# phuang1024/Starst3r

Hardware: AMD Instinct MI355X
Metric: 3DGS train iters/sec @ 1M Gaussians, 8x1080p views (higher is better)
Workload: dtype f32

## Files before the change

### starst3r_amd/csrc/api.hip

```cpp
#include <stdarg.h>

#include "common.h"

static thread_local char g_err[512] = "";

void st3r_set_error(const char* fmt, ...) {
    va_list ap;
    va_start(ap, fmt);
    vsnprintf(g_err, sizeof(g_err), fmt, ap);
    va_end(ap);
}

ST3R_EXPORT int st3r_version(void) { return ST3R_VERSION; }
ST3R_EXPORT const char* st3r_last_error(void) { return g_err; }

ST3R_EXPORT int st3r_ctx_create(int device, st3r_ctx** out) {
    ARG_CHECK(out);
    int ndev = 0;
    HIP_TRY(hipGetDeviceCount(&ndev));
    ARG_CHECK(device >= 0 && device < ndev);
    HIP_TRY(hipSetDevice(device));
    st3r_ctx* c = new (std::nothrow) st3r_ctx();
    if (!c) { st3r_set_error("out of host memory"); return ST3R_ERR_NOMEM; }
    memset(c, 0, sizeof(*c));
// ... 43 lines not shown
    *grown = 0;
    if (bytes == 0) bytes = 16;
    if (ctx->slot_bytes[slot] < bytes) {
        size_t want = bytes + bytes / 4;
        want = (want + 255) & ~(size_t)255;
        if (ctx->slot_ptr[slot]) {
            HIP_TRY(hipDeviceSynchronize());
            HIP_TRY(hipFree(ctx->slot_ptr[slot]));
            ctx->slot_ptr[slot] = nullptr; ctx->slot_bytes[slot] = 0;
        }
        hipError_t e = hipMalloc(&ctx->slot_ptr[slot], want);
        if (e != hipSuccess) {
            st3r_set_error("arena slot %d: hipMalloc(%zu) failed: %s", slot, want, hipGetErrorString(e));
            return ST3R_ERR_NOMEM;
        }
        ctx->slot_bytes[slot] = want;
        *grown = 1;
    }
    *out = ctx->slot_ptr[slot];
    return ST3R_OK;
}

ST3R_EXPORT int st3r_ctx_peek(st3r_ctx* ctx, void* stream, int which, void* dst, int64_t bytes) {
    ARG_CHECK(ctx && dst && bytes >= 0 && which >= 0 && which <= 10);
    static const int slots[11] = {SLOT_VALS_B, SLOT_OFFSETS, SLOT_SPLATS, SLOT_CUM,
                                  SLOT_MCMC_CUM, SLOT_MCMC_DEAD, SLOT_MCMC_SAMPLED, SLOT_MCMC_COUNT,
                                  SLOT_RGB, SLOT_ALPHA, SLOT_COUNTS};
    ARG_CHECK((size_t)bytes <= ctx->slot_bytes[slots[which]]);
    HIP_TRY(hipMemcpyAsync(dst, ctx->slot_ptr[slots[which]], (size_t)bytes, hipMemcpyDeviceToDevice,
                           (hipStream_t)stream));
    return ST3R_OK;
}

static const char* k_stage_names[STG_COUNT] = {"project", "scan", "emit", "sort", "offsets", "blend_fwd", "loss",
                                               "blend_bwd", "project_bwd", "adam", "sort_depth"};

ST3R_EXPORT const char* st3r_stage_name(int stage) {
    return (stage >= 0 && stage < STG_COUNT) ? k_stage_names[stage] : "";
}

static void prof_harvest_slot(st3r_ctx* ctx, int slot) {
    for (int st = 0; st < STG_COUNT; ++st) {
        if (!ctx->prof_used[slot][st]) continue;
        float ms = 0.f;
        if (hipEventSynchronize(ctx->prof_ev[slot][st][1]) == hipSuccess &&
            hipEventElapsedTime(&ms, ctx->prof_ev[slot][st][0], ctx->prof_ev[slot][st][1]) == hipSuccess) {
            ctx->prof_ms[st] += ms; ctx->prof_n[st] += 1;
        }
        ctx->prof_used[slot][st] = 0;
    }
// ... 43 lines not shown
        ctx->prof_ms[st] = 0; ctx->prof_n[st] = 0;
    }
    return ST3R_OK;
}

int st3r_isect_scan_impl(st3r_ctx* ctx, hipStream_t s, int64_t n_pairs, const int32_t* tiles, int32_t* cum,
                         int64_t* n_isects_host, const void* pack_rects, int rect32, uint64_t* pack_out,
                         int32_t** total_dev_out, int32_t* total_copy, int32_t* total_host);
int st3r_isect_emit_impl(hipStream_t s, int N, int C, const float* splats, const int32_t* cum, int tile_size,
                         int tile_w, int tile_h, int64_t* isect_ids, int32_t* flatten_ids);
int st3r_sort_impl(st3r_ctx* ctx, hipStream_t s, int64_t n, int end_bit, int64_t* keys_in, int32_t* vals_in,
                   int64_t* keys_out, int32_t* vals_out);
int st3r_isect_offsets_impl(hipStream_t s, int64_t n_isects, const int64_t* ids, int C, int tile_w, int tile_h,
                            int32_t* offsets);
int st3r_project_impl(st3r_ctx* ctx, hipStream_t s, int N, int C, const float* means, const float* quats, const float* scales,
                      const float* opacities, const float* sh, int sh_stride, const float* viewmats, const float* Ks,
                      const float* campos, int width, int height, int tile_size, float eps2d, float near_plane,
                      float far_plane, float radius_clip, float* splats, int32_t* tiles_per_gauss, double* reg_sums,
                      uint64_t* depth_keys, int32_t* depth_vals, int tight, uint32_t key_base, void* rects, int rect32,
                      int reg_overwrite, double* zero_ptr, int zero_n, uint32_t* krange);
int st3r_sort_depth_seg_impl(st3r_ctx* ctx, hipStream_t s, int64_t N, int C, uint32_t* keys_in, int32_t* vals_in,
                             uint32_t* keys_out, int32_t* vals_out, const uint32_t* krange);
int st3r_isect_emit_chain_impl(st3r_ctx* ctx, hipStream_t s, int N, int C, const int32_t* perm, const void* rects,
                               int rect32, int tile_w, int tile_h, uint32_t* tile_keys, int32_t* vals, int64_t cap);
int st3r_records_prepare_impl(hipStream_t s, int N, int C, const float* splats, int tile_size, int tile_w, int tile_h,
                              int tight, int32_t* tiles, uint64_t* depth_keys, int32_t* depth_vals, uint32_t key_base,
                              void* rects, int rect32);
int st3r_isect_offsets32_impl(hipStream_t s, int64_t n_isects, const uint32_t* keys, int C, int tile_w, int tile_h,
                              int32_t* offsets, const int32_t* n_dev);
int st3r_sort_depth_impl(st3r_ctx* ctx, hipStream_t s, int64_t n, int end_bit, uint64_t* keys_in, int32_t* vals_in,
                         uint64_t* keys_out, int32_t* vals_out);
int st3r_sort_depth32_impl(st3r_ctx* ctx, hipStream_t s, int64_t n, int end_bit, uint32_t* keys_in, int32_t* vals_in,
                           uint32_t* keys_out, int32_t* vals_out);
int st3r_sort_tile_impl(st3r_ctx* ctx, hipStream_t s, int64_t n, int end_bit, uint32_t* keys_in, int32_t* vals_in,
                        uint32_t* keys_out, int32_t* vals_out, const int32_t* n_dev);
int st3r_blend_fwd_impl(st3r_ctx* ctx, hipStream_t s, int C, int W, int H, int tile_w, int tile_h,
                        const float* splats, const int32_t* offsets, const int32_t* flat, int64_t n_isects,
                        float* rgb, float* alpha, int32_t* last_ids, bool for_backward, bool end_in_offsets);
int st3r_blend_bwd_impl(st3r_ctx* ctx, hipStream_t s, int C, int W, int H, int tile_w, int tile_h,
                        const float* splats, const int32_t* offsets, const int32_t* flat, int64_t n_isects,
                        const float* alpha, const int32_t* last_ids, const float* v_rgb, const float* v_alpha,
                        const int32_t* cum, const uint64_t* rects, const uint64_t* rectbase, int tight, int64_t n_pairs,
                        float* v_splats,
                        bool end_in_offsets, st3r_vtile_ref* defer);
int st3r_project_sh_bwd_impl(hipStream_t s, int N, int C, const float* means, const float* quats, const float* scales,
                             const float* opacities, const float* sh, int sh_stride, const float* viewmats,
                             const float* Ks, const float* campos, int width, int height, float eps2d,
// ... 144 lines not shown
        if (n_isects > 2147483647LL) n_isects = 2147483647LL;
        ctx->count_pending = 1; ctx->count_cap = n_isects;
        o->n_visible = -1; o->n_isects_ref = -1;
    } else {
        HIP_TRY(hipMemcpyAsync(ctx->pinned, total_dev, sizeof(int32_t), hipMemcpyDeviceToHost, s));
        if (reg_sums) HIP_TRY(hipMemcpyAsync(ctx->pinned + 1, reg_sums + 2, 2 * sizeof(double), hipMemcpyDeviceToHost, s));
        HIP_TRY(hipStreamSynchronize(s));
        n_isects = (int64_t)((int32_t*)ctx->pinned)[0];
        if (n_isects < 0) {
            st3r_set_error("more than 2^31 tile intersections in one call: split the views over more calls / GPUs");
            return ST3R_SPLIT_VIEWS;
        }
        o->n_visible = reg_sums ? (int64_t)((double*)ctx->pinned)[1] : -1;
        o->n_isects_ref = reg_sums ? (int64_t)((double*)ctx->pinned)[2] : n_isects;
        if (allow_async) { ctx->isect_hint = n_isects; ctx->hint_sig = sig; }
    }
    GET(SLOT_KEYS_A, uint32_t, n_isects, tkeys_a);
    GET(SLOT_KEYS_B, uint32_t, n_isects, tkeys_b);
    GET(SLOT_VALS_A, int32_t, n_isects, vals_a);
    GET(SLOT_VALS_B, int32_t, n_isects, vals_b);
    n_dev = total_dev;
    o->n_records = async ? -1 : n_isects;
    if (n_isects > 0) {
        st3r_prof_begin(ctx, s, STG_EMIT);
        rc = st3r_isect_emit_chain_impl(ctx, s, N, C, perm, rects, rect32, tile_w, tile_h, tkeys_a, vals_a, n_isects);
        st3r_prof_end(ctx, s, STG_EMIT);
        if (rc) return rc;
        const int end_bit = bit_length_u32((uint32_t)((int64_t)C * tile_w * tile_h - 1));
        st3r_prof_begin(ctx, s, STG_SORT);
        rc = st3r_sort_tile_impl(ctx, s, n_isects, end_bit, tkeys_a, vals_a, tkeys_b, vals_b, n_dev);
        st3r_prof_end(ctx, s, STG_SORT);
        if (rc) return rc;
    }
    st3r_prof_begin(ctx, s, STG_OFFSETS);
    rc = st3r_isect_offsets32_impl(s, n_isects, tkeys_b, C, tile_w, tile_h, offsets, n_dev);
    st3r_prof_end(ctx, s, STG_OFFSETS);
    if (rc) return rc;
    o->splats = splats; o->offsets = offsets; o->flat = vals_b; o->cum = cum; o->rects = rect32 ? nullptr : rects;
    o->rectbase = rectbase;
    o->n_isects = n_isects;
    o->tile_w = tile_w; o->tile_h = tile_h;
    return ST3R_OK;
}

__global__ void k_finalize_loss(int C, const double* __restrict__ sums, const double* __restrict__ reg_sums,
                                double inv_px, double inv_cnt, double w_l1, double w_ssim, double reg_views,
                                double opac_k, double scale_k, float* __restrict__ loss_out) {
    if (threadIdx.x == 0 && blockIdx.x == 0) {
        double loss = 0;
        for (int c = 0; c < C; ++c) loss += w_l1 * sums[2 * c] * inv_px + w_ssim * (1.0 - sums[2 * c + 1] * inv_cnt);
        loss += reg_views * (opac_k * reg_sums[0] + scale_k * reg_sums[1]);
        loss_out[0] = (float)loss;
    }
// ... 192 lines not shown
```

### starst3r_amd/csrc/common.h

```cpp
#pragma once
#include <hip/hip_runtime.h>
#include <stdint.h>
#include <stdio.h>
#include <string.h>

#include "../../include/st3r.h"

#define ST3R_EXPORT extern "C" __attribute__((visibility("default")))

void st3r_set_error(const char* fmt, ...);

#define HIP_TRY(expr)                                                                              \
    do {                                                                                           \
        hipError_t _e = (expr);                                                                    \
        if (_e != hipSuccess) {                                                                    \
            st3r_set_error("%s:%d: %s -> %s", __FILE__, __LINE__, #expr, hipGetErrorString(_e));   \
            return ST3R_ERR_HIP;                                                                   \
        }                                                                                          \
    } while (0)

#define ARG_CHECK(cond)                                                                    \
    do {                                                                                   \
        if (!(cond)) {                                                                     \
            st3r_set_error("%s:%d: invalid argument: %s", __FILE__, __LINE__, #cond);      \
// ... 28 lines not shown
    SLOT_DKEYS_B,
    SLOT_DVALS_A,
    SLOT_DVALS_B,
    SLOT_CUM_D,
    SLOT_NN_PART,
    SLOT_MCMC_CUM,
    SLOT_MCMC_DEAD,
    SLOT_MCMC_RANK,
    SLOT_MCMC_COUNT,
    SLOT_MCMC_SAMPLED,
    SLOT_MCMC_BINOMS,
    SLOT_REG_PART,
    SLOT_RECTS,
    SLOT_RECTS_D,
    SLOT_RECTBASE,
    SLOT_COUNTS,
    SLOT_PSTAGE,
    SLOT_GSTAGE,
    SLOT_ALIGN_CTL,
    SLOT_PAIR_TOUCH,
    SLOT_KRANGE_PART,
    SLOT_SCAN_CHAIN,
    SLOT_POSE_PART,
    SLOT_COUNT
};

enum Stage {
    STG_PROJECT = 0,
    STG_SCAN,
    STG_EMIT,
    STG_SORT,
    STG_OFFSETS,
    STG_BLEND_FWD,
    STG_LOSS,
    STG_BLEND_BWD,
    STG_PROJECT_BWD,
    STG_ADAM,
    STG_SORT_DEPTH,
    STG_COUNT
};
#define PROF_RING 64
#define ST3R_MAX_RANGES 8

#define ST3R_SPLIT_VIEWS 1000

struct st3r_vtile_ref { const int32_t* cum; const float* vtile; int stamp; unsigned vt_cap; const uint32_t* touch; };
// ... 44 lines not shown
```

### starst3r_amd/csrc/gs_isect.hip

```cpp
#include "common.h"
#include "tile_rect.h"

#define SCAN_THREADS 256
#define SCAN_ITEMS 16
#define SCAN_TILE (SCAN_THREADS * SCAN_ITEMS)

__device__ __forceinline__ int wave_incl_scan(int v) {
    const int lane = threadIdx.x & 63;
#pragma unroll
    for (int off = 1; off < 64; off <<= 1) {
        int t = __shfl_up(v, off);
        if (lane >= off) v += t;
    }
    return v;
}

__device__ __forceinline__ int block_incl_scan(int v, int* total) {
    __shared__ int wsum[4];
    const int lane = threadIdx.x & 63, w = threadIdx.x >> 6;
    int inc = wave_incl_scan(v);
    if (lane == 63) wsum[w] = inc;
    __syncthreads();
    int base = 0;
#pragma unroll
// ... 357 lines not shown
                              void* rects, int rect32) {
    const int64_t n_pairs = (int64_t)N * C;
    if (n_pairs == 0) return ST3R_OK;
    hipLaunchKernelGGL(k_records_prepare, dim3(ceil_div(n_pairs, 256)), dim3(256), 0, s, N, n_pairs,
                       (const float4*)splats, tile_size, tile_w, tile_h, tight, tiles, depth_keys, depth_vals, key_base,
                       rects, rect32);
    LAUNCH_CHECK();
    return ST3R_OK;
}


#ifndef EP
#define EP 1024
#endif
#define EPT (EP / 256)
#define ECH 4096

__device__ __forceinline__ void emit_item(int C, int bpc, int* c, int* k) {
    const int b = blockIdx.x;
    if ((C & 7) == 0) { const int j = b >> 3; *c = (b & 7) + 8 * (j / bpc); *k = j % bpc; }
    else { *c = b / bpc; *k = b % bpc; }
}

__global__ __launch_bounds__(256) void k_isect_gather(int N, int C, int bpc, const int32_t* __restrict__ perm,
                                                      const void* __restrict__ rects, int rect32,
                                                      void* __restrict__ rects_d, int32_t* __restrict__ wg_tiles) {
    int c, k;
    emit_item(C, bpc, &c, &k);
    const int t = threadIdx.x;
    const int64_t first = (int64_t)c * N + (int64_t)k * EP;
    const int np = (int)min((int64_t)EP, (int64_t)(c + 1) * N - first);
    int32_t pid[EPT];
#pragma unroll
    for (int j = 0; j < EPT; ++j) pid[j] = j * 256 + t < np ? perm[first + j * 256 + t] : -1;
    int sum = 0;
#pragma unroll
    for (int j = 0; j < EPT; ++j) {
        if (pid[j] >= 0) {
            const int64_t dst = first + j * 256 + t;
            if (rect32) {
                const uint32_t r = reinterpret_cast<const uint32_t*>(rects)[pid[j]];
                reinterpret_cast<uint32_t*>(rects_d)[dst] = r;
                sum += (int)((r >> 16) & 0xFFu) * (int)(r >> 24);
            } else {
                const uint64_t r = reinterpret_cast<const uint64_t*>(rects)[pid[j]];
                reinterpret_cast<uint64_t*>(rects_d)[dst] = r;
                sum += (int)((r >> 32) & 0xFFFF) * (int)(r >> 48);
            }
        }
    }
    int total;
    block_incl_scan(sum, &total);
    if (t == 0) wg_tiles[c * bpc + k] = total;
}

#define EMIT_SELF_BASE_MAX 16384
__global__ __launch_bounds__(1024) void k_isect_wg_scan(int n, const int32_t* __restrict__ wg_tiles,
                                                        long long* __restrict__ wg_base) {
    __shared__ long long s_wave[16];
    const int t = threadIdx.x, lane = t & 63, w = t >> 6;
    const int per = (n + 1023) / 1024;
    const int e0 = min(t * per, n), e1 = min(e0 + per, n);
    long long sum = 0;
    for (int e = e0; e < e1; ++e) sum += wg_tiles[e];
    long long inc = sum;
#pragma unroll
    for (int off = 1; off < 64; off <<= 1) {
        const long long o = __shfl_up(inc, off);
        if (lane >= off) inc += o;
    }
    if (lane == 63) s_wave[w] = inc;
    __syncthreads();
    long long base = 0;
#pragma unroll
    for (int i = 0; i < 16; ++i) base += i < w ? s_wave[i] : 0;
    long long run = base + inc - sum;
    for (int e = e0; e < e1; ++e) { wg_base[e] = run; run += wg_tiles[e]; }
}

__global__ __launch_bounds__(256) void k_isect_emit_d(int N, int C, int bpc, const int32_t* __restrict__ perm,
                                                      const void* __restrict__ rects_d, int rect32,
                                                      const long long* __restrict__ wg_base,
                                                      const int32_t* __restrict__ wg_tiles, int tile_w, int tile_h,
                                                      uint32_t* __restrict__ tile_keys, int32_t* __restrict__ vals,
                                                      int64_t cap) {
    __shared__ int s_end[EP];
    __shared__ uint32_t s_org[EP];
    __shared__ uint16_t s_w[EP];
    __shared__ int32_t s_pid[EP];
    __shared__ uint16_t s_own[ECH];
    __shared__ unsigned s_wmax[4];
    __shared__ long long s_bsum[4];
    int c, k;
    emit_item(C, bpc, &c, &k);
    const int t = threadIdx.x, lane = t & 63, w = t >> 6;
    long long bsum = 0;
    if (!wg_base) {
        const int nb4 = (c * bpc + k) >> 2;
        for (int i = t; i < nb4; i += 256) {
            const int4 v = reinterpret_cast<const int4*>(wg_tiles)[i];
            bsum += ((long long)v.x + v.y) + ((long long)v.z + v.w);
        }
        if (t < ((c * bpc + k) & 3)) bsum += wg_tiles[4 * nb4 + t];
    }
    const int64_t first = (int64_t)c * N + (int64_t)k * EP;
    const int np = (int)min((int64_t)EP, (int64_t)(c + 1) * N - first);
    int cnt[EPT];
#pragma unroll
    for (int j = 0; j < EPT; ++j) {
        const int e = j * 256 + t;
        int32_t pid = 0;
        uint32_t org = 0, rw = 0, rh = 0;
        if (e < np) {
            pid = perm[first + e];
            rect_load(rects_d, rect32, first + e, &org, &rw, &rh);
        }
        s_pid[e] = pid; s_org[e] = org; s_w[e] = (uint16_t)rw;
        cnt[j] = (int)(rw * rh);
    }
    int carry = 0;
#pragma unroll
    for (int j = 0; j < EPT; ++j) {
        int tot;
        const int inc = block_incl_scan(cnt[j], &tot);
        s_end[j * 256 + t] = carry + inc;
        carry += tot;
    }
    const int total = carry;
    __syncthreads();
    long long base;
    if (wg_base) base = wg_base[c * bpc + k];
    else {
#pragma unroll
        for (int off = 32; off > 0; off >>= 1) bsum += __shfl_down(bsum, off);
        if (lane == 0) s_bsum[w] = bsum;
        __syncthreads();
        base = (s_bsum[0] + s_bsum[1]) + (s_bsum[2] + s_bsum[3]);
    }
    const uint32_t key0 = (uint32_t)c * (uint32_t)(tile_w * tile_h);
    int carry_owner = 0;
    for (int c0 = 0; c0 < total; c0 += ECH) {
        reinterpret_cast<uint4*>(s_own)[t] = make_uint4(0u, 0u, 0u, 0u);
        reinterpret_cast<uint4*>(s_own)[t + 256] = make_uint4(0u, 0u, 0u, 0u);
        __syncthreads();
#pragma unroll
        for (int j = 0; j < EPT; ++j) {
            const int e = j * 256 + t;
            if (e < np) {
                const int start = e ? s_end[e - 1] : 0;
                if (s_end[e] > start && start >= c0 && start < c0 + ECH) s_own[start - c0] = (uint16_t)(e + 1);
            }
        }
        __syncthreads();
        uint4 a = reinterpret_cast<const uint4*>(s_own)[2 * t], b = reinterpret_cast<const uint4*>(s_own)[2 * t + 1];
        unsigned wv[8] = {a.x, a.y, a.z, a.w, b.x, b.y, b.z, b.w};
        unsigned run = 0;
#pragma unroll
        for (int i = 0; i < 8; ++i) {
            const unsigned lo = max(run, wv[i] & 0xFFFFu);
            run = max(lo, wv[i] >> 16);
            wv[i] = lo | (run << 16);
        }
        unsigned inc = run;
#pragma unroll
        for (int off = 1; off < 64; off <<= 1) {
            const unsigned o = __shfl_up(inc, off);
            if (lane >= off) inc = max(inc, o);
        }
        if (lane == 63) s_wmax[w] = inc;
        unsigned excl_m = __shfl_up(inc, 1);
        if (lane == 0) excl_m = 0;
        __syncthreads();
        unsigned pre = max((unsigned)carry_owner, excl_m);
#pragma unroll
        for (int ww = 0; ww < 4; ++ww)
            if (ww < w) pre = max(pre, s_wmax[ww]);
        carry_owner = (int)max(max(max((unsigned)carry_owner, s_wmax[0]), max(s_wmax[1], s_wmax[2])), s_wmax[3]);
#pragma unroll
        for (int i = 0; i < 8; ++i) {
            const unsigned lo = max(wv[i] & 0xFFFFu, pre), hi = max(wv[i] >> 16, pre);
            wv[i] = lo | (hi << 16);
        }
        reinterpret_cast<uint4*>(s_own)[2 * t] = make_uint4(wv[0], wv[1], wv[2], wv[3]);
        reinterpret_cast<uint4*>(s_own)[2 * t + 1] = make_uint4(wv[4], wv[5], wv[6], wv[7]);
        __syncthreads();
        const int lim = min(ECH, total - c0);
        for (int i = t; i < lim; i += 256) {
            const int p = (int)s_own[i] - 1;
            const int o = c0 + i;
            const int kk = o - (p == 0 ? 0 : s_end[p - 1]);
            const uint32_t w_ = s_w[p], org = s_org[p];
            int qq = (int)((float)kk * __builtin_amdgcn_rcpf((float)w_));
            int rem = kk - qq * (int)w_;
            if (rem < 0) { --qq; rem += (int)w_; }
            if (rem >= (int)w_) { ++qq; rem -= (int)w_; }
            const uint32_t tx = (org & 0xFFFF) + (uint32_t)rem, ty = (org >> 16) + (uint32_t)qq;
            const long long pos = base + o;
            if (pos >= 0 && pos < cap) {
                tile_keys[pos] = key0 + ty * (uint32_t)tile_w + tx;
                vals[pos] = s_pid[p];
            }
        }
        __syncthreads();
    }
}

int st3r_isect_emit_chain_impl(st3r_ctx* ctx, hipStream_t s, int N, int C, const int32_t* perm, const void* rects,
                               int rect32, int tile_w, int tile_h, uint32_t* tile_keys, int32_t* vals, int64_t cap) {
    const int64_t n_pairs = (int64_t)N * C;
    if (n_pairs == 0) return ST3R_OK;
    const int bpc = ceil_div(N, EP);
    const int grid = C * bpc;
    void* p;
    int rc = st3r_arena_get(ctx, SLOT_RECTS_D, (rect32 ? sizeof(uint32_t) : sizeof(uint64_t)) * (size_t)n_pairs, &p);
    if (rc) return rc;
    void* rects_d = p;
    rc = st3r_arena_get(ctx, SLOT_CUM_D, (sizeof(long long) + sizeof(int32_t)) * (size_t)grid + 16, &p);
    if (rc) return rc;
    long long* wg_base = (long long*)p;
    int32_t* wg_tiles = (int32_t*)(wg_base + grid);
    if (((uintptr_t)wg_tiles & 15) != 0) wg_tiles += 2;
    hipLaunchKernelGGL(k_isect_gather, dim3(grid), dim3(256), 0, s, N, C, bpc, perm, rects, rect32, rects_d, wg_tiles);
    const bool self_base = grid <= EMIT_SELF_BASE_MAX;
    if (!self_base) hipLaunchKernelGGL(k_isect_wg_scan, dim3(1), dim3(1024), 0, s, grid, wg_tiles, wg_base);
    hipLaunchKernelGGL(k_isect_emit_d, dim3(grid), dim3(256), 0, s, N, C, bpc, perm, rects_d, rect32,
                       self_base ? (const long long*)nullptr : wg_base, wg_tiles, tile_w, tile_h, tile_keys, vals, cap);
    LAUNCH_CHECK();
    return ST3R_OK;
}
```

### starst3r_amd/csrc/radix_sort.h

```cpp
#pragma once
#include "common.h"

int st3r_radix_sort_u32(st3r_ctx* ctx, hipStream_t s, int64_t n, int begin_bit, int end_bit, const uint32_t* keys_in,
                        const int32_t* vals_in, uint32_t* keys_out, int32_t* vals_out);
int st3r_radix_sort_u64(st3r_ctx* ctx, hipStream_t s, int64_t n, int begin_bit, int end_bit, const uint64_t* keys_in,
                        const int32_t* vals_in, uint64_t* keys_out, int32_t* vals_out);
int st3r_radix_sort_u32_devcount(st3r_ctx* ctx, hipStream_t s, int64_t n_cap, const int32_t* n_dev, int begin_bit,
                                 int end_bit, const uint32_t* keys_in, const int32_t* vals_in, uint32_t* keys_out,
                                 int32_t* vals_out);
int st3r_radix_sort_u32_segments(st3r_ctx* ctx, hipStream_t s, int64_t seg_n, int n_seg, const uint32_t* keys_in,
                                 const int32_t* vals_in, uint32_t* keys_out, int32_t* vals_out, const uint32_t* krange);
```

### starst3r_amd/csrc/radix_sort.hip

```cpp
#include "radix_sort.h"

namespace {

constexpr int RB = 8;
constexpr int RADIX = 1 << RB;
#ifndef RS_THREADS
#define RS_THREADS 1024
#endif
#ifndef RS_SMALL_BELOW
#define RS_SMALL_BELOW 100
#endif
constexpr int THREADS_L = RS_THREADS, THREADS_S = 512;
constexpr int HIST_THREADS = 256;
constexpr int HIST_ITEMS = 16;
constexpr int MAX_PASSES = 8;
constexpr int HIST_COPIES = 8;

typedef unsigned long long u64;
constexpr u64 FLAG_AGG = 1ull << 62, FLAG_INC = 2ull << 62, VALUE_MASK = (1ull << 62) - 1;

template <typename K> struct Traits;
#ifndef RS_IPT32
#define RS_IPT32 16
#endif
template <> struct Traits<uint32_t> { static constexpr int IPT = RS_IPT32, IPT_S = 8; };
template <> struct Traits<uint64_t> { static constexpr int IPT = 8, IPT_S = 4; };

__device__ __forceinline__ int wave_incl_scan_u32(uint32_t v, int lane) {
#pragma unroll
    for (int off = 1; off < 64; off <<= 1) {
        const uint32_t t = __shfl_up(v, off);
        if (lane >= off) v += t;
    }
    return v;
}

__device__ __forceinline__ uint32_t pair_lane_u32(uint32_t v, int q) {
    return q == 0 ? (uint32_t)__builtin_amdgcn_mov_dpp((int)v, 0xA0, 0xf, 0xf, true)
                  : (uint32_t)__builtin_amdgcn_mov_dpp((int)v, 0xF5, 0xf, 0xf, true);
// ... 71 lines not shown
                const uint32_t kk = seg_key(k[i], kmin, ktop);
                for (int p = 0; p < passes; ++p) atomicAdd(&mine[p * RADIX + ((kk >> (RB * p)) & (RADIX - 1))], 1u);
            }
        }
    }
    __syncthreads();
    for (int i = threadIdx.x; i < passes * RADIX; i += HIST_THREADS) {
        uint32_t t = 0;
#pragma unroll
        for (int w = 0; w < HIST_THREADS / 64; ++w) t += sh[w][i];
        if (t) atomicAdd(&hist[blockIdx.y * (MAX_PASSES * RADIX) + i], t);
    }
}

template <typename K, int THREADS, int IPT, bool SEG = false>
__global__ __launch_bounds__(THREADS) void k_rs_pass(const K* __restrict__ kin, const int32_t* __restrict__ vin,
                                                     K* __restrict__ kout, int32_t* __restrict__ vout, int64_t n,
                                                     int shift, int bits, const uint32_t* __restrict__ hist_base,
                                                     u64* status, uint32_t* tile_counter,
                                                     const int32_t* __restrict__ n_dev, int64_t seg_n = 0,
                                                     int tiles_per_seg = 0, const uint32_t* __restrict__ krange = nullptr,
                                                     int ps = 0, K* __restrict__ ktmp = nullptr,
                                                     int32_t* __restrict__ vtmp = nullptr) {
    if (n_dev) n = min(n, (int64_t)max(*n_dev, 0));
    constexpr int TILE = THREADS * IPT, WAVES = THREADS / 64;
    uint32_t kmin = 0, ktop = 0;
    bool last_seg_pass = false;
    if constexpr (SEG) {
        const int np = (int)krange[2];
        last_seg_pass = ps == np - 1;
        if (ps >= np) return;
        const bool to_out = ((np - 1 - ps) & 1) == 0;
        const K* src_k = ps == 0 ? kin : (to_out ? ktmp : kout);
        const int32_t* src_v = ps == 0 ? vin : (to_out ? vtmp : vout);
        K* dst_k = to_out ? kout : ktmp;
        int32_t* dst_v = to_out ? vout : vtmp;
        kin = src_k; vin = src_v; kout = dst_k; vout = dst_v;
        kmin = krange[0]; ktop = krange[1];
        shift = RB * ps; bits = RB;
    }
    __shared__ K sbuf[TILE];
    __shared__ int32_t svals[TILE];
    __shared__ uint32_t whist[WAVES][RADIX];
    __shared__ uint32_t lbase[RADIX];
    __shared__ uint32_t tcnt[RADIX];
    __shared__ u64 gexc[RADIX];
// ... 135 lines not shown
        }
    }
    __syncthreads();
    if (tid < RADIX) gofs[tid] = (long long)((u64)hexc + gexc[tid]) - (long long)lbase[tid] + seg_base;
    __syncthreads();

#pragma unroll
    for (int i = 0; i < IPT; ++i) {
        if (wbase + i * 64 < tcount) {
            const uint32_t d = (uint32_t)(key[i] >> shift) & dmask;
            const uint32_t pos = lbase[d] + wh[d] + rank[i];
            sbuf[pos] = key[i];
            if (has_vals) svals[pos] = val[i];
        }
    }
    __syncthreads();
#pragma unroll
    for (int i = 0; i < IPT; ++i) {
        const int p = i * THREADS + tid;
        if (p < tcount) {
            const K k = sbuf[p];
            const uint32_t d = (uint32_t)(k >> shift) & dmask;
            const long long o = gofs[d] + p;
            if (!(SEG && last_seg_pass)) kout[o] = k;
            if (has_vals) vout[o] = svals[p];
        }
    }
}

inline size_t align256(size_t v) { return (v + 255) & ~(size_t)255; }

template <typename K>
int sort_pairs(st3r_ctx* ctx, hipStream_t s, int64_t n, int begin_bit, int end_bit, const K* keys_in,
               const int32_t* vals_in, K* keys_out, int32_t* vals_out, const int32_t* n_dev = nullptr) {
    if (n == 0) return ST3R_OK;
    if (end_bit > (int)sizeof(K) * 8) end_bit = (int)sizeof(K) * 8;
    if (begin_bit < 0 || begin_bit >= end_bit) { st3r_set_error("radix sort: empty bit range"); return ST3R_ERR_INVALID; }
    const int passes = (end_bit - begin_bit + RB - 1) / RB;
    constexpr int TILE_L = THREADS_L * Traits<K>::IPT, TILE_S = THREADS_S * Traits<K>::IPT_S;
    const bool small = (n + TILE_L - 1) / TILE_L < RS_SMALL_BELOW;
    const int64_t TILE = small ? TILE_S : TILE_L;
    const int64_t ntiles = (n + TILE - 1) / TILE;
    const size_t hist_bytes = align256(sizeof(uint32_t) * (size_t)(HIST_COPIES * MAX_PASSES * RADIX + MAX_PASSES));
    const size_t status_bytes = sizeof(u64) * (size_t)passes * (size_t)ntiles * RADIX;
    const size_t meta_bytes = hist_bytes + align256(status_bytes);
    const bool need_tmp = passes > 1;
    const size_t tk_bytes = need_tmp ? align256(sizeof(K) * (size_t)n) : 0;
    const size_t tv_bytes = need_tmp && vals_in ? align256(sizeof(int32_t) * (size_t)n) : 0;
// ... 56 lines not shown
    uint32_t* counters = hist + (size_t)n_seg * MAX_PASSES * RADIX;
    u64* status = (u64*)(base + hist_bytes);
    K* tk = (K*)(base + meta_bytes);
    int32_t* tv = (int32_t*)(base + meta_bytes + tk_bytes);
    HIP_TRY(hipMemsetAsync(base, 0, meta_bytes, s));
    const int hist_blocks = (int)std::max<int64_t>(1, std::min<int64_t>(1024 / n_seg, (seg_n + HIST_THREADS * HIST_ITEMS - 1) / (HIST_THREADS * HIST_ITEMS)));
    hipLaunchKernelGGL(k_rs_hist_seg, dim3(hist_blocks, n_seg), dim3(HIST_THREADS), 0, s, keys_in, seg_n, hist, krange);
    for (int ps = 0; ps < PASSES; ++ps) {
        if (small)
            hipLaunchKernelGGL((k_rs_pass<K, THREADS_S, Traits<K>::IPT_S, true>), dim3((unsigned)ntiles), dim3(THREADS_S), 0, s,
                               keys_in, vals_in, keys_out, vals_out, n, 0, RB, hist + ps * RADIX,
                               status + (size_t)ps * ntiles * RADIX, counters + ps, (const int32_t*)nullptr, seg_n,
                               tiles_per_seg, krange, ps, tk, tv);
        else
            hipLaunchKernelGGL((k_rs_pass<K, THREADS_L, Traits<K>::IPT, true>), dim3((unsigned)ntiles), dim3(THREADS_L), 0, s,
                               keys_in, vals_in, keys_out, vals_out, n, 0, RB, hist + ps * RADIX,
                               status + (size_t)ps * ntiles * RADIX, counters + ps, (const int32_t*)nullptr, seg_n,
                               tiles_per_seg, krange, ps, tk, tv);
    }
    LAUNCH_CHECK();
    return ST3R_OK;
}

}

int st3r_radix_sort_u32_segments(st3r_ctx* ctx, hipStream_t s, int64_t seg_n, int n_seg, const uint32_t* keys_in,
                                 const int32_t* vals_in, uint32_t* keys_out, int32_t* vals_out, const uint32_t* krange) {
    return sort_pairs_seg(ctx, s, seg_n, n_seg, keys_in, vals_in, keys_out, vals_out, krange);
}

int st3r_radix_sort_u32(st3r_ctx* ctx, hipStream_t s, int64_t n, int begin_bit, int end_bit, const uint32_t* keys_in,
                        const int32_t* vals_in, uint32_t* keys_out, int32_t* vals_out) {
    return sort_pairs<uint32_t>(ctx, s, n, begin_bit, end_bit, keys_in, vals_in, keys_out, vals_out);
}

int st3r_radix_sort_u64(st3r_ctx* ctx, hipStream_t s, int64_t n, int begin_bit, int end_bit, const uint64_t* keys_in,
                        const int32_t* vals_in, uint64_t* keys_out, int32_t* vals_out) {
    return sort_pairs<uint64_t>(ctx, s, n, begin_bit, end_bit, keys_in, vals_in, keys_out, vals_out);
}

int st3r_radix_sort_u32_devcount(st3r_ctx* ctx, hipStream_t s, int64_t n_cap, const int32_t* n_dev, int begin_bit,
                                 int end_bit, const uint32_t* keys_in, const int32_t* vals_in, uint32_t* keys_out,
                                 int32_t* vals_out) {
    return sort_pairs<uint32_t>(ctx, s, n_cap, begin_bit, end_bit, keys_in, vals_in, keys_out, vals_out, n_dev);
}
```

Measured before the change: 193.1.

## Fuse first radix-sort pass of tile keys into intersection emit kernel

When tile keys fit in 9 to 16 bits, the gather kernel now builds per-workgroup low-digit and high-digit histograms directly from tile rectangles. A new digit-base kernel turns these into per-workgroup scatter offsets. The emit kernel then ranks keys by low digit in shared memory and scatters them straight into low-digit-sorted order, so the sort only needs the second pass. This removes one full read/write pass plus a histogram pass over the intersection keys. In exchange it adds per-block atomics, a per-workgroup histogram buffer and extra shared-memory staging in emit.

New measurement: 195.0, median of 6. +1.0%, better.

```diff
diff --git a/starst3r_amd/csrc/api.hip b/starst3r_amd/csrc/api.hip
--- a/starst3r_amd/csrc/api.hip
+++ b/starst3r_amd/csrc/api.hip
@@ -89,10 +89,10 @@
 }
 
 ST3R_EXPORT int st3r_ctx_peek(st3r_ctx* ctx, void* stream, int which, void* dst, int64_t bytes) {
-    ARG_CHECK(ctx && dst && bytes >= 0 && which >= 0 && which <= 10);
-    static const int slots[11] = {SLOT_VALS_B, SLOT_OFFSETS, SLOT_SPLATS, SLOT_CUM,
+    ARG_CHECK(ctx && dst && bytes >= 0 && which >= 0 && which <= 11);
+    static const int slots[12] = {SLOT_VALS_B, SLOT_OFFSETS, SLOT_SPLATS, SLOT_CUM,
                                   SLOT_MCMC_CUM, SLOT_MCMC_DEAD, SLOT_MCMC_SAMPLED, SLOT_MCMC_COUNT,
-                                  SLOT_RGB, SLOT_ALPHA, SLOT_COUNTS};
+                                  SLOT_RGB, SLOT_ALPHA, SLOT_COUNTS, SLOT_KEYS_B};
     ARG_CHECK((size_t)bytes <= ctx->slot_bytes[slots[which]]);
     HIP_TRY(hipMemcpyAsync(dst, ctx->slot_ptr[slots[which]], (size_t)bytes, hipMemcpyDeviceToDevice,
                            (hipStream_t)stream));
@@ -182,7 +182,10 @@
 int st3r_sort_depth_seg_impl(st3r_ctx* ctx, hipStream_t s, int64_t N, int C, uint32_t* keys_in, int32_t* vals_in,
                              uint32_t* keys_out, int32_t* vals_out, const uint32_t* krange);
 int st3r_isect_emit_chain_impl(st3r_ctx* ctx, hipStream_t s, int N, int C, const int32_t* perm, const void* rects,
-                               int rect32, int tile_w, int tile_h, uint32_t* tile_keys, int32_t* vals, int64_t cap);
+                               int rect32, int tile_w, int tile_h, uint32_t* tile_keys, int32_t* vals, int64_t cap,
+                               int fuse_end_bit, int* fused);
+int st3r_tile_sort_fused_pass(st3r_ctx* ctx, hipStream_t s, int64_t n_cap, const int32_t* n_dev, int end_bit,
+                              const uint32_t* keys_in, const int32_t* vals_in, uint32_t* keys_out, int32_t* vals_out);
 int st3r_records_prepare_impl(hipStream_t s, int N, int C, const float* splats, int tile_size, int tile_w, int tile_h,
                               int tight, int32_t* tiles, uint64_t* depth_keys, int32_t* depth_vals, uint32_t key_base,
                               void* rects, int rect32);
@@ -373,13 +376,16 @@
     n_dev = total_dev;
     o->n_records = async ? -1 : n_isects;
     if (n_isects > 0) {
+        const int end_bit = bit_length_u32((uint32_t)((int64_t)C * tile_w * tile_h - 1));
+        int fused = 0;
         st3r_prof_begin(ctx, s, STG_EMIT);
-        rc = st3r_isect_emit_chain_impl(ctx, s, N, C, perm, rects, rect32, tile_w, tile_h, tkeys_a, vals_a, n_isects);
+        rc = st3r_isect_emit_chain_impl(ctx, s, N, C, perm, rects, rect32, tile_w, tile_h, tkeys_a, vals_a, n_isects,
+                                        (ctx->debug_flags & 16) ? 0 : end_bit, &fused);
         st3r_prof_end(ctx, s, STG_EMIT);
         if (rc) return rc;
-        const int end_bit = bit_length_u32((uint32_t)((int64_t)C * tile_w * tile_h - 1));
         st3r_prof_begin(ctx, s, STG_SORT);
-        rc = st3r_sort_tile_impl(ctx, s, n_isects, end_bit, tkeys_a, vals_a, tkeys_b, vals_b, n_dev);
+        rc = fused ? st3r_tile_sort_fused_pass(ctx, s, n_isects, n_dev, end_bit, tkeys_a, vals_a, tkeys_b, vals_b)
+                   : st3r_sort_tile_impl(ctx, s, n_isects, end_bit, tkeys_a, vals_a, tkeys_b, vals_b, n_dev);
         st3r_prof_end(ctx, s, STG_SORT);
         if (rc) return rc;
     }
diff --git a/starst3r_amd/csrc/common.h b/starst3r_amd/csrc/common.h
--- a/starst3r_amd/csrc/common.h
+++ b/starst3r_amd/csrc/common.h
@@ -74,6 +74,7 @@
     SLOT_KRANGE_PART,
     SLOT_SCAN_CHAIN,
     SLOT_POSE_PART,
+    SLOT_WG_DIGITS,
     SLOT_COUNT
 };
 
diff --git a/starst3r_amd/csrc/gs_isect.hip b/starst3r_amd/csrc/gs_isect.hip
--- a/starst3r_amd/csrc/gs_isect.hip
+++ b/starst3r_amd/csrc/gs_isect.hip
@@ -1,5 +1,6 @@
 #include "common.h"
 #include "tile_rect.h"
+#include "radix_sort.h"
 
 #define SCAN_THREADS 256
 #define SCAN_ITEMS 16
@@ -403,36 +404,142 @@
     else { *c = b / bpc; *k = b % bpc; }
 }
 
+template <bool DIGITS>
 __global__ __launch_bounds__(256) void k_isect_gather(int N, int C, int bpc, const int32_t* __restrict__ perm,
                                                       const void* __restrict__ rects, int rect32,
-                                                      void* __restrict__ rects_d, int32_t* __restrict__ wg_tiles) {
+                                                      void* __restrict__ rects_d, int32_t* __restrict__ wg_tiles,
+                                                      int tile_w, int tile_h, uint32_t* __restrict__ wg_hist,
+                                                      uint32_t* __restrict__ hist) {
+    __shared__ int s_diff[DIGITS ? 256 : 1];
+    __shared__ uint32_t s_hi[DIGITS ? 256 : 1];
+    __shared__ uint32_t s_full;
     int c, k;
     emit_item(C, bpc, &c, &k);
     const int t = threadIdx.x;
+    if (DIGITS) {
+        s_diff[t] = 0; s_hi[t] = 0;
+        if (t == 0) s_full = 0;
+    }
     const int64_t first = (int64_t)c * N + (int64_t)k * EP;
     const int np = (int)min((int64_t)EP, (int64_t)(c + 1) * N - first);
     int32_t pid[EPT];
 #pragma unroll
     for (int j = 0; j < EPT; ++j) pid[j] = j * 256 + t < np ? perm[first + j * 256 + t] : -1;
     int sum = 0;
+    uint32_t org[EPT], rw[EPT], rh[EPT];
 #pragma unroll
     for (int j = 0; j < EPT; ++j) {
+        org[j] = 0; rw[j] = 0; rh[j] = 0;
         if (pid[j] >= 0) {
             const int64_t dst = first + j * 256 + t;
             if (rect32) {
                 const uint32_t r = reinterpret_cast<const uint32_t*>(rects)[pid[j]];
                 reinterpret_cast<uint32_t*>(rects_d)[dst] = r;
                 sum += (int)((r >> 16) & 0xFFu) * (int)(r >> 24);
+                if (DIGITS) { org[j] = (r & 0xFFu) | ((r & 0xFF00u) << 8); rw[j] = (r >> 16) & 0xFFu; rh[j] = r >> 24; }
             } else {
                 const uint64_t r = reinterpret_cast<const uint64_t*>(rects)[pid[j]];
                 reinterpret_cast<uint64_t*>(rects_d)[dst] = r;
                 sum += (int)((r >> 32) & 0xFFFF) * (int)(r >> 48);
+                if (DIGITS) { org[j] = (uint32_t)r; rw[j] = (uint32_t)(r >> 32) & 0xFFFFu; rh[j] = (uint32_t)(r >> 48); }
             }
         }
+    }
+    if (DIGITS) {
+        __syncthreads();
+        const uint32_t key0 = (uint32_t)c * (uint32_t)(tile_w * tile_h);
+        uint32_t full = 0;
+#pragma unroll
+        for (int j = 0; j < EPT; ++j) {
+            const uint32_t w = rw[j];
+            if (w == 0) continue;
+            uint32_t kr = key0 + (org[j] >> 16) * (uint32_t)tile_w + (org[j] & 0xFFFFu);
+            const uint32_t rem = w & 255u;
+            for (uint32_t r = 0; r < rh[j]; ++r, kr += (uint32_t)tile_w) {
+                full += w >> 8;
+                const uint32_t lo = kr & 255u;
+                if (rem) {
+                    atomicAdd(&s_diff[lo], 1);
+                    const uint32_t e = lo + rem;
+                    if (e < 256u) atomicAdd(&s_diff[e], -1);
+                    else if (e > 256u) { atomicAdd(&s_diff[0], 1); atomicAdd(&s_diff[e - 256u], -1); }
+                }
+                const uint32_t kl = kr + w - 1u, h1 = kl >> 8;
+                uint32_t h0 = kr >> 8;
+                if (h0 == h1) atomicAdd(&s_hi[h0], w);
+                else {
+                    atomicAdd(&s_hi[h0], 256u - lo);
+                    for (++h0; h0 < h1; ++h0) atomicAdd(&s_hi[h0], 256u);
+                    atomicAdd(&s_hi[h1], (kl & 255u) + 1u);
+                }
+            }
+        }
+        if (full) atomicAdd(&s_full, full);
     }
     int total;
     block_incl_scan(sum, &total);
     if (t == 0) wg_tiles[c * bpc + k] = total;
+    if (DIGITS) {
+        int tot;
+        const uint32_t cnt = s_full + (uint32_t)block_incl_scan(s_diff[t], &tot);
+        wg_hist[(size_t)(c * bpc + k) * 256 + t] = cnt;
+        uint32_t* const hc = hist + (blockIdx.x & (RS_HIST_COPIES - 1)) * RS_HIST_STRIDE;
+        if (cnt) atomicAdd(hc + t, cnt);
+        const uint32_t hh = s_hi[t];
+        if (hh) atomicAdd(hc + 256 + t, hh);
+    }
+}
+
+#define DB_THREADS 1024
+__global__ __launch_bounds__(DB_THREADS) void k_isect_digit_base(int grid, uint32_t* __restrict__ wg_hist,
+                                                                 const uint32_t* __restrict__ hist) {
+    __shared__ uint32_t s_h[256];
+    __shared__ uint32_t s_low[4];
+    __shared__ uint4 s_wv[DB_THREADS / 64];
+    const int b = blockIdx.x, g = (b & 7) * 8 + (b >> 3);
+    const int t = threadIdx.x, lane = t & 63, w = t >> 6;
+    const int per = (grid + DB_THREADS - 1) / DB_THREADS;
+    const int r0 = min(t * per, grid), r1 = min(r0 + per, grid);
+    uint4* const col = reinterpret_cast<uint4*>(wg_hist) + g;
+    uint4 sum = make_uint4(0u, 0u, 0u, 0u);
+#pragma unroll 8
+    for (int r = r0; r < r1; ++r) {
+        const uint4 v = col[(size_t)r * 64];
+        sum.x += v.x; sum.y += v.y; sum.z += v.z; sum.w += v.w;
+    }
+    if (t < 256) {
+        uint32_t hv = 0;
+#pragma unroll
+        for (int cc = 0; cc < RS_HIST_COPIES; ++cc) hv += hist[cc * RS_HIST_STRIDE + t];
+        s_h[t] = hv;
+        uint32_t below = t < 4 * g ? hv : 0u;
+#pragma unroll
+        for (int off = 32; off > 0; off >>= 1) below += __shfl_xor(below, off);
+        if (lane == 0) s_low[w] = below;
+    }
+    uint4 inc = sum;
+#pragma unroll
+    for (int off = 1; off < 64; off <<= 1) {
+        const uint32_t ox = __shfl_up(inc.x, off), oy = __shfl_up(inc.y, off), oz = __shfl_up(inc.z, off),
+                       ow = __shfl_up(inc.w, off);
+        if (lane >= off) { inc.x += ox; inc.y += oy; inc.z += oz; inc.w += ow; }
+    }
+    if (lane == 63) s_wv[w] = inc;
+    __syncthreads();
+    const uint32_t gb = (s_low[0] + s_low[1]) + (s_low[2] + s_low[3]);
+    uint4 run = make_uint4(gb, gb + s_h[4 * g], gb + s_h[4 * g] + s_h[4 * g + 1],
+                           gb + s_h[4 * g] + s_h[4 * g + 1] + s_h[4 * g + 2]);
+    for (int ww = 0; ww < w; ++ww) {
+        const uint4 o = s_wv[ww];
+        run.x += o.x; run.y += o.y; run.z += o.z; run.w += o.w;
+    }
+    run.x += inc.x - sum.x; run.y += inc.y - sum.y; run.z += inc.z - sum.z; run.w += inc.w - sum.w;
+#pragma unroll 8
+    for (int r = r0; r < r1; ++r) {
+        const uint4 v = col[(size_t)r * 64];
+        col[(size_t)r * 64] = run;
+        run.x += v.x; run.y += v.y; run.z += v.z; run.w += v.w;
+    }
 }
 
 #define EMIT_SELF_BASE_MAX 16384
@@ -459,24 +566,128 @@
     for (int e = e0; e < e1; ++e) { wg_base[e] = run; run += wg_tiles[e]; }
 }
 
+#ifndef EMIT_FUSED_MODE
+#define EMIT_FUSED_MODE 2
+#endif
+__device__ __forceinline__ void emit_decode(int i, int c0, uint32_t key0, int tile_w, const uint16_t* s_own,
+                                            const int* s_end, const uint16_t* s_w, const uint32_t* s_org, uint32_t* key,
+                                            uint32_t* p_out) {
+    const int p = (int)s_own[i] - 1;
+    const int o = c0 + i;
+    const int kk = o - (p == 0 ? 0 : s_end[p - 1]);
+    const uint32_t w_ = s_w[p], org = s_org[p];
+    int qq = (int)((float)kk * __builtin_amdgcn_rcpf((float)w_));
+    int rem = kk - qq * (int)w_;
+    if (rem < 0) { --qq; rem += (int)w_; }
+    if (rem >= (int)w_) { ++qq; rem -= (int)w_; }
+    const uint32_t tx = (org & 0xFFFF) + (uint32_t)rem, ty = (org >> 16) + (uint32_t)qq;
+    *key = key0 + ty * (uint32_t)tile_w + tx;
+    *p_out = (uint32_t)p;
+}
+
+template <int MODE>
+__device__ __forceinline__ void emit_chunk_ranked(int lim, int c0, uint32_t key0, int tile_w, const uint16_t* s_own,
+                                                  const int* s_end, const uint16_t* s_w, const uint32_t* s_org,
+                                                  const int32_t* s_pid, uint32_t (*s_wh)[256], uint32_t* s_db,
+                                                  uint32_t* s_lb, uint32_t* s_buf, uint32_t* __restrict__ tile_keys,
+                                                  int32_t* __restrict__ vals, int64_t cap) {
+    const int t = threadIdx.x, lane = t & 63, w = t >> 6;
+    constexpr int ROWS = ECH / 256;
+    uint32_t pk[ROWS], rk[ROWS];
+    uint32_t* const wh = s_wh[w];
+    const uint64_t lt = (1ull << lane) - 1ull;
+#pragma unroll
+    for (int j = 0; j < ROWS; ++j) {
+        const int i = w * (ECH / 4) + j * 64 + lane;
+        const bool valid = i < lim;
+        uint32_t key = 0, p = 0;
+        if (valid) emit_decode(i, c0, key0, tile_w, s_own, s_end, s_w, s_org, &key, &p);
+        pk[j] = key | (p << 16);
+        const uint32_t d = key & 255u;
+        uint64_t m = __ballot(valid);
+#pragma unroll
+        for (int bt = 0; bt < 8; ++bt) {
+            const bool bit = (d >> bt) & 1u;
+            const uint64_t bal = __ballot(bit);
+            m &= bit ? bal : ~bal;
+        }
+        const uint32_t below = (uint32_t)__popcll(m & lt);
+        const uint32_t prev = wh[d];
+        if (valid && below == 0) wh[d] = prev + (uint32_t)__popcll(m);
+        rk[j] = prev + below;
+    }
+    __syncthreads();
+    uint32_t cnt = 0;
+#pragma unroll
+    for (int ww = 0; ww < 4; ++ww) {
+        const uint32_t x = s_wh[ww][t];
+        s_wh[ww][t] = cnt;
+        cnt += x;
+    }
+    if (MODE == 2) {
+        int tot;
+        s_lb[t] = (uint32_t)block_incl_scan((int)cnt, &tot) - cnt;
+    }
+    __syncthreads();
+    if (MODE == 1) {
+#pragma unroll
+        for (int j = 0; j < ROWS; ++j) {
+            if (w * (ECH / 4) + j * 64 + lane < lim) {
+                const uint32_t d = pk[j] & 255u;
+                const long long pos = (long long)s_db[d] + s_wh[w][d] + rk[j];
+                if (pos < cap) {
+                    tile_keys[pos] = pk[j] & 0xFFFFu;
+                    vals[pos] = s_pid[pk[j] >> 16];
+                }
+            }
+        }
+    } else {
+#pragma unroll
+        for (int j = 0; j < ROWS; ++j) {
+            if (w * (ECH / 4) + j * 64 + lane < lim) {
+                const uint32_t d = pk[j] & 255u;
+                s_buf[s_lb[d] + s_wh[w][d] + rk[j]] = pk[j];
+            }
+        }
+        __syncthreads();
+        for (int q = t; q < lim; q += 256) {
+            const uint32_t v = s_buf[q], d = v & 255u;
+            const long long pos = (long long)s_db[d] + (uint32_t)(q - (int)s_lb[d]);
+            if (pos < cap) {
+                tile_keys[pos] = v & 0xFFFFu;
+                vals[pos] = s_pid[v >> 16];
+            }
+        }
+    }
+    __syncthreads();
+    s_db[t] += cnt;
+}
+
+template <int MODE>
 __global__ __launch_bounds__(256) void k_isect_emit_d(int N, int C, int bpc, const int32_t* __restrict__ perm,
                                                       const void* __restrict__ rects_d, int rect32,
                                                       const long long* __restrict__ wg_base,
                                                       const int32_t* __restrict__ wg_tiles, int tile_w, int tile_h,
                                                       uint32_t* __restrict__ tile_keys, int32_t* __restrict__ vals,
-                                                      int64_t cap) {
+                                                      int64_t cap, const uint32_t* __restrict__ dbase) {
+    constexpr bool FUSED = MODE != 0;
     __shared__ int s_end[EP];
     __shared__ uint32_t s_org[EP];
     __shared__ uint16_t s_w[EP];
     __shared__ int32_t s_pid[EP];
-    __shared__ uint16_t s_own[ECH];
+    __shared__ uint32_t s_buf[MODE == 2 ? ECH : ECH / 2];
+    uint16_t* const s_own = reinterpret_cast<uint16_t*>(s_buf);
     __shared__ unsigned s_wmax[4];
     __shared__ long long s_bsum[4];
+    __shared__ uint32_t s_wh[FUSED ? 4 : 1][256];
+    __shared__ uint32_t s_db[FUSED ? 256 : 1];
+    __shared__ uint32_t s_lb[MODE == 2 ? 256 : 1];
     int c, k;
     emit_item(C, bpc, &c, &k);
     const int t = threadIdx.x, lane = t & 63, w = t >> 6;
+    if (FUSED) s_db[t] = dbase[(size_t)(c * bpc + k) * 256 + t];
     long long bsum = 0;
-    if (!wg_base) {
+    if (!FUSED && !wg_base) {
         const int nb4 = (c * bpc + k) >> 2;
         for (int i = t; i < nb4; i += 256) {
             const int4 v = reinterpret_cast<const int4*>(wg_tiles)[i];
@@ -509,8 +720,9 @@
     }
     const int total = carry;
     __syncthreads();
-    long long base;
-    if (wg_base) base = wg_base[c * bpc + k];
+    long long base = 0;
+    if (FUSED) {
+    } else if (wg_base) base = wg_base[c * bpc + k];
     else {
 #pragma unroll
         for (int off = 32; off > 0; off >>= 1) bsum += __shfl_down(bsum, off);
@@ -523,6 +735,10 @@
     for (int c0 = 0; c0 < total; c0 += ECH) {
         reinterpret_cast<uint4*>(s_own)[t] = make_uint4(0u, 0u, 0u, 0u);
         reinterpret_cast<uint4*>(s_own)[t + 256] = make_uint4(0u, 0u, 0u, 0u);
+        if (FUSED) {
+#pragma unroll
+            for (int i = 0; i < 4; ++i) (&s_wh[0][0])[i * 256 + t] = 0u;
+        }
         __syncthreads();
 #pragma unroll
         for (int j = 0; j < EPT; ++j) {
@@ -566,6 +782,11 @@
         reinterpret_cast<uint4*>(s_own)[2 * t + 1] = make_uint4(wv[4], wv[5], wv[6], wv[7]);
         __syncthreads();
         const int lim = min(ECH, total - c0);
+        if (FUSED) {
+            emit_chunk_ranked<MODE>(lim, c0, key0, tile_w, s_own, s_end, s_w, s_org, s_pid, s_wh, s_db, s_lb, s_buf,
+                                    tile_keys, vals, cap);
+            continue;
+        }
         for (int i = t; i < lim; i += 256) {
             const int p = (int)s_own[i] - 1;
             const int o = c0 + i;
@@ -586,8 +807,11 @@
     }
 }
 
+
 int st3r_isect_emit_chain_impl(st3r_ctx* ctx, hipStream_t s, int N, int C, const int32_t* perm, const void* rects,
-                               int rect32, int tile_w, int tile_h, uint32_t* tile_keys, int32_t* vals, int64_t cap) {
+                               int rect32, int tile_w, int tile_h, uint32_t* tile_keys, int32_t* vals, int64_t cap,
+                               int fuse_end_bit, int* fused) {
+    *fused = 0;
     const int64_t n_pairs = (int64_t)N * C;
     if (n_pairs == 0) return ST3R_OK;
     const int bpc = ceil_div(N, EP);
@@ -601,11 +825,30 @@
     long long* wg_base = (long long*)p;
     int32_t* wg_tiles = (int32_t*)(wg_base + grid);
     if (((uintptr_t)wg_tiles & 15) != 0) wg_tiles += 2;
-    hipLaunchKernelGGL(k_isect_gather, dim3(grid), dim3(256), 0, s, N, C, bpc, perm, rects, rect32, rects_d, wg_tiles);
     const bool self_base = grid <= EMIT_SELF_BASE_MAX;
+    if (self_base && fuse_end_bit > 8 && fuse_end_bit <= 16) {
+        uint32_t* hist = nullptr;
+        rc = st3r_tile_sort_fused_prepare(ctx, s, cap, &hist);
+        if (rc) return rc;
+        rc = st3r_arena_get(ctx, SLOT_WG_DIGITS, sizeof(uint32_t) * 256 * (size_t)grid, &p);
+        if (rc) return rc;
+        uint32_t* wg_hist = (uint32_t*)p;
+        hipLaunchKernelGGL(k_isect_gather<true>, dim3(grid), dim3(256), 0, s, N, C, bpc, perm, rects, rect32, rects_d,
+                           wg_tiles, tile_w, tile_h, wg_hist, hist);
+        hipLaunchKernelGGL(k_isect_digit_base, dim3(64), dim3(DB_THREADS), 0, s, grid, wg_hist, (const uint32_t*)hist);
+        hipLaunchKernelGGL(k_isect_emit_d<EMIT_FUSED_MODE>, dim3(grid), dim3(256), 0, s, N, C, bpc, perm, rects_d, rect32,
+                           (const long long*)nullptr, wg_tiles, tile_w, tile_h, tile_keys, vals, cap,
+                           (const uint32_t*)wg_hist);
+        LAUNCH_CHECK();
+        *fused = 1;
+        return ST3R_OK;
+    }
+    hipLaunchKernelGGL(k_isect_gather<false>, dim3(grid), dim3(256), 0, s, N, C, bpc, perm, rects, rect32, rects_d,
+                       wg_tiles, tile_w, tile_h, (uint32_t*)nullptr, (uint32_t*)nullptr);
     if (!self_base) hipLaunchKernelGGL(k_isect_wg_scan, dim3(1), dim3(1024), 0, s, grid, wg_tiles, wg_base);
-    hipLaunchKernelGGL(k_isect_emit_d, dim3(grid), dim3(256), 0, s, N, C, bpc, perm, rects_d, rect32,
-                       self_base ? (const long long*)nullptr : wg_base, wg_tiles, tile_w, tile_h, tile_keys, vals, cap);
+    hipLaunchKernelGGL(k_isect_emit_d<0>, dim3(grid), dim3(256), 0, s, N, C, bpc, perm, rects_d, rect32,
+                       self_base ? (const long long*)nullptr : wg_base, wg_tiles, tile_w, tile_h, tile_keys, vals, cap,
+                       (const uint32_t*)nullptr);
     LAUNCH_CHECK();
     return ST3R_OK;
 }
diff --git a/starst3r_amd/csrc/radix_sort.h b/starst3r_amd/csrc/radix_sort.h
--- a/starst3r_amd/csrc/radix_sort.h
+++ b/starst3r_amd/csrc/radix_sort.h
@@ -8,5 +8,10 @@
 int st3r_radix_sort_u32_devcount(st3r_ctx* ctx, hipStream_t s, int64_t n_cap, const int32_t* n_dev, int begin_bit,
                                  int end_bit, const uint32_t* keys_in, const int32_t* vals_in, uint32_t* keys_out,
                                  int32_t* vals_out);
+#define RS_HIST_COPIES 8
+#define RS_HIST_STRIDE 2048
+int st3r_tile_sort_fused_prepare(st3r_ctx* ctx, hipStream_t s, int64_t n_cap, uint32_t** hist);
+int st3r_tile_sort_fused_pass(st3r_ctx* ctx, hipStream_t s, int64_t n_cap, const int32_t* n_dev, int end_bit,
+                              const uint32_t* keys_in, const int32_t* vals_in, uint32_t* keys_out, int32_t* vals_out);
 int st3r_radix_sort_u32_segments(st3r_ctx* ctx, hipStream_t s, int64_t seg_n, int n_seg, const uint32_t* keys_in,
                                  const int32_t* vals_in, uint32_t* keys_out, int32_t* vals_out, const uint32_t* krange);
diff --git a/starst3r_amd/csrc/radix_sort.hip b/starst3r_amd/csrc/radix_sort.hip
--- a/starst3r_amd/csrc/radix_sort.hip
+++ b/starst3r_amd/csrc/radix_sort.hip
@@ -15,6 +15,7 @@
 constexpr int HIST_ITEMS = 16;
 constexpr int MAX_PASSES = 8;
 constexpr int HIST_COPIES = 8;
+static_assert(HIST_COPIES == RS_HIST_COPIES && MAX_PASSES * RADIX == RS_HIST_STRIDE, "histogram layout of radix_sort.h");
 
 typedef unsigned long long u64;
 constexpr u64 FLAG_AGG = 1ull << 62, FLAG_INC = 2ull << 62, VALUE_MASK = (1ull << 62) - 1;
@@ -132,6 +133,7 @@
                                                      int tiles_per_seg = 0, const uint32_t* __restrict__ krange = nullptr,
                                                      int ps = 0, K* __restrict__ ktmp = nullptr,
                                                      int32_t* __restrict__ vtmp = nullptr) {
+    const int64_t n_cap = n;
     if (n_dev) n = min(n, (int64_t)max(*n_dev, 0));
     constexpr int TILE = THREADS * IPT, WAVES = THREADS / 64;
     uint32_t kmin = 0, ktop = 0;
@@ -313,8 +315,10 @@
             const K k = sbuf[p];
             const uint32_t d = (uint32_t)(k >> shift) & dmask;
             const long long o = gofs[d] + p;
-            if (!(SEG && last_seg_pass)) kout[o] = k;
-            if (has_vals) vout[o] = svals[p];
+            if (o < n_cap) {
+                if (!(SEG && last_seg_pass)) kout[o] = k;
+                if (has_vals) vout[o] = svals[p];
+            }
         }
     }
 }
@@ -417,6 +421,57 @@
     return ST3R_OK;
 }
 
+struct FusedMeta { uint32_t* hist; uint32_t* counter; u64* status; int64_t ntiles; bool small; size_t bytes; };
+inline FusedMeta fused_meta_layout(int64_t n_cap) {
+    typedef uint32_t K;
+    constexpr int TILE_L = THREADS_L * Traits<K>::IPT, TILE_S = THREADS_S * Traits<K>::IPT_S;
+    FusedMeta m{};
+    m.small = (n_cap + TILE_L - 1) / TILE_L < RS_SMALL_BELOW;
+    m.ntiles = (n_cap + (m.small ? TILE_S : TILE_L) - 1) / (m.small ? TILE_S : TILE_L);
+    const size_t hist_bytes = align256(sizeof(uint32_t) * (size_t)(HIST_COPIES * MAX_PASSES * RADIX + MAX_PASSES));
+    m.bytes = hist_bytes + align256(sizeof(u64) * (size_t)m.ntiles * RADIX);
+    return m;
+}
+inline int fused_meta(st3r_ctx* ctx, int64_t n_cap, FusedMeta* m) {
+    *m = fused_meta_layout(n_cap);
+    void* p;
+    const int rc = st3r_arena_get(ctx, SLOT_SORT_TMP, m->bytes, &p);
+    if (rc) return rc;
+    m->hist = (uint32_t*)p;
+    m->counter = m->hist + HIST_COPIES * MAX_PASSES * RADIX;
+    m->status = (u64*)((char*)p + align256(sizeof(uint32_t) * (size_t)(HIST_COPIES * MAX_PASSES * RADIX + MAX_PASSES)));
+    return ST3R_OK;
+}
+
+}
+
+int st3r_tile_sort_fused_prepare(st3r_ctx* ctx, hipStream_t s, int64_t n_cap, uint32_t** hist) {
+    FusedMeta m;
+    int rc = fused_meta(ctx, n_cap, &m);
+    if (rc) return rc;
+    HIP_TRY(hipMemsetAsync(m.hist, 0, m.bytes, s));
+    *hist = m.hist;
+    return ST3R_OK;
+}
+
+int st3r_tile_sort_fused_pass(st3r_ctx* ctx, hipStream_t s, int64_t n_cap, const int32_t* n_dev, int end_bit,
+                              const uint32_t* keys_in, const int32_t* vals_in, uint32_t* keys_out, int32_t* vals_out) {
+    if (n_cap == 0) return ST3R_OK;
+    if (end_bit <= RB || end_bit > 2 * RB) { st3r_set_error("fused tile sort: end_bit %d outside (8, 16]", end_bit); return ST3R_ERR_INVALID; }
+    FusedMeta m;
+    int rc = fused_meta(ctx, n_cap, &m);
+    if (rc) return rc;
+    typedef uint32_t K;
+    if (m.small)
+        hipLaunchKernelGGL((k_rs_pass<K, THREADS_S, Traits<K>::IPT_S>), dim3((unsigned)m.ntiles), dim3(THREADS_S), 0, s,
+                           keys_in, vals_in, keys_out, vals_out, n_cap, RB, end_bit - RB, m.hist + RADIX, m.status,
+                           m.counter, n_dev);
+    else
+        hipLaunchKernelGGL((k_rs_pass<K, THREADS_L, Traits<K>::IPT>), dim3((unsigned)m.ntiles), dim3(THREADS_L), 0, s,
+                           keys_in, vals_in, keys_out, vals_out, n_cap, RB, end_bit - RB, m.hist + RADIX, m.status,
+                           m.counter, n_dev);
+    LAUNCH_CHECK();
+    return ST3R_OK;
 }
 
 int st3r_radix_sort_u32_segments(st3r_ctx* ctx, hipStream_t s, int64_t seg_n, int n_seg, const uint32_t* keys_in,
```
